# theori-io/nrsc5

Hardware: NVIDIA H100
Metric: cu8 I/Q Msamples/s (higher is better)
Workload: dtype u8/int16/f32

## Files before the change

### nrsc5_b200/csrc/common.cuh

```cuda
#pragma once
#include <cuda_runtime.h>
#include <stdint.h>

namespace nb {

constexpr int NFFT = 2048;
constexpr int NCP = 112;
constexpr int NSYM = NFFT + NCP;
constexpr int BLK = 32;
constexpr int NACQ = NSYM * (BLK + 1);
constexpr int LB0 = NFFT / 2 - 546;
constexpr int UB1 = NFFT / 2 + 546;
constexpr int PW = 19;
constexpr int MAXPART = 14;
constexpr int SIDE = MAXPART * PW + 1;
constexpr int NBINS = 2 * SIDE;
constexpr int PM_BLOCK = 23040;
constexpr int P1_LEN = 146176;
constexpr int P1_ENC = P1_LEN * 5 / 2;
constexpr int P1_VIT = P1_LEN * 3;
constexpr int P1_STEPS = P1_LEN + 64;
constexpr int PIDS_LEN = 80;
constexpr int P3_LEN = 4608;
constexpr int IV_N = 147456;
// ... 23 lines not shown
                   REC_BER = 6, REC_SOFT_PM = 8, REC_BLOCK = 9, REC_PAD = 12;

__host__ __device__ inline int compact_of_bin(int b)
{
    if (b >= LB0 && b < LB0 + SIDE) return b - LB0;
    if (b > UB1 - SIDE && b <= UB1) return SIDE + (b - (UB1 - SIDE + 1));
    return -1;
}

constexpr int L2_QUEUE = 40;

struct StreamState {
    long long in_avail;
    long long start;
    float prev_angle;
    float2 phase;
    int keep_extra;
    int cfo;
    int state;
    int samperr;
    float angle;
    int psmi, cfo_wait, bc, mer_cnt;
    float err_lb, err_ub;
    int started_pm;
    int active;
    int blk_samperr;
    int blk_state_in;
    int blk_go;
    float theta;
    float2 phase0;
    int p1_ready;
    int p1_slow;
    int p1_retry;
    unsigned p1_rec;
    unsigned p1_lost_rec;
    int p1_errs;
    int p1_done;
    int pids_pending;
    int pids_bc[16];
    unsigned pids_rec[16];
    long long px_total[2];
    int px_started[2];
    int xq_pending[PX_GROUPS];
    long long xq_k0[PX_GROUPS][P3_SLOTS];
    unsigned xq_rec[PX_GROUPS][P3_SLOTS];
    int force_state;
    int l2_n;
    unsigned l2_off[L2_QUEUE], l2_lc[L2_QUEUE], l2_nbits[L2_QUEUE];
    unsigned log_len;
    unsigned log_overflow;
    unsigned long long blocks_done;
    unsigned long long frames_done;
    unsigned long long p1_fallbacks;
    unsigned long long ph_cyc[6];
    unsigned long long ph_n[6];
    unsigned long long sy_cyc[6];
    short bp_hist[31][2];
    short bp_hist_next[31][2];
};

struct EngineDims {
    int nstreams;
    size_t in_stride;
    size_t log_cap;
    int emit_soft;
    int cs16;
    int px_enabled;
    int l2;
    int cluster;
};

struct PxBufs {
    int8_t *vin;
    uint2 *dec;
    uint32_t *spec, *end;
    int *endstate;
    uint2 *fspec, *fend;
    int *fhstate, *ftbend;
    uint32_t *bits;
    int *flags;
};

struct EngineCtl {
    unsigned long long progress;
    unsigned px_need;
    unsigned more;
};

struct StreamBrief {
    long long start;
    int state, bc, p1_ready, pad_;
};

struct DevPtrs {
    EngineCtl *ctl;
    StreamBrief *brief;
    const uint8_t *iq;
    StreamState *st;
    float *cfreq;
    float *cphase;
    float2 *nco;
    float2 *bins;
    int8_t *pm;
    short2 *ydec;
    float2 *acq_sums;
    float2 *tbuf;
    int8_t *vit_in;
    uint2 *vit_dec;
    uint32_t *p1_bits;
    uint2 *vspec, *vend;
    int *hstate, *tbend;
    uint32_t *v64_spec, *v64_end;
    int *v64_endstate;
    int8_t *px_ring[2];
    const uint32_t *iv_delay;
    const uint32_t *iv_delay_s;
    PxBufs xb[PX_GROUPS];
    uint8_t *log;
    const float *shape;
    const float2 *twid;
    const uint32_t *p1_lut;
    const uint8_t *pn;
    const uint32_t *pnw;
};

__device__ inline uint8_t *log_reserve(const DevPtrs &p, const EngineDims &d, int s, uint32_t type, uint32_t plen)
{
    StreamState &st = p.st[s];
    uint32_t need = 8 + ((plen + 3) & ~3u);
    if ((size_t)st.log_len + need > d.log_cap) {
        st.log_overflow = 1;
        return nullptr;
    }
    uint8_t *w = p.log + (size_t)s * d.log_cap + st.log_len;
    reinterpret_cast<uint32_t *>(w)[0] = type;
    reinterpret_cast<uint32_t *>(w)[1] = plen;
    st.log_len += need;
    return w + 8;
}

__device__ __forceinline__ void l2_enqueue(StreamState &st, int l2_on, unsigned off, unsigned lc, unsigned nbits)
{
    if (!l2_on) return;
    if (st.l2_n >= L2_QUEUE) {
        st.log_overflow = 1;
        return;
    }
    const int e = st.l2_n++;
    st.l2_off[e] = off;
    st.l2_lc[e] = lc;
    st.l2_nbits[e] = nbits;
}

template <int R>
__device__ __forceinline__ void halfband_run(const uint32_t *w, short2 *y)
{
    const int tap[4] = { -134, 1078, -4417, 19864 };
    int lr[R + 7], li[R + 7];
    int cr[R], ci[R];
#pragma unroll
    for (int q = 0; q < R + 7; q++) {
        const uint32_t v = w[q];
        lr[q] = (int)(v & 0xffu);
        li[q] = (int)((v >> 8) & 0xffu);
        if (q >= 3 && q < R + 3) {
            cr[q - 3] = (int)((v >> 16) & 0xffu);
            ci[q - 3] = (int)(v >> 24);
        }
    }
#pragma unroll
    for (int r = 0; r < R; r++) {
        int ar = cr[r] * 64 - 127 * 64, ai = ci[r] * 64 - 127 * 64;
#pragma unroll
        for (int k = 0; k < 4; k++) {
            ar += ((lr[r + k] + lr[r + 7 - k]) * tap[k] - 254 * tap[k]) >> 9;
            ai += ((li[r + k] + li[r + 7 - k]) * tap[k] - 254 * tap[k]) >> 9;
        }
        y[r] = make_short2((short)ar, (short)ai);
    }
}

}
```

### nrsc5_b200/csrc/front.cuh

```cuda
#pragma once
#include "pids_crc.cuh"
#include "common.cuh"
#include "fft.cuh"
#include "viterbi_pack.cuh"

namespace nb {

constexpr int FRONT_THREADS = 1024;
constexpr int TEAMS = FRONT_THREADS / 128;
constexpr int MAXREF = 15;
constexpr int IN_BYTES = 4 * NSYM + 28 + 16 + 16;
constexpr int IN_STRIDE = 8704;
constexpr int ACQ_TILE = 4096;

__device__ int g_dbg;

__constant__ int c_compat_mode[64];
__constant__ unsigned c_pn80[3];
__constant__ short c_bp_tap[32];

__device__ __forceinline__ float2 cmulf(float2 a, float2 b)
{
    return make_float2(a.x * b.x - a.y * b.y, a.x * b.y + a.y * b.x);
}
__device__ __forceinline__ float2 cexp_j(float a)
{
    float s, c;
    sincosf(a, &s, &c);
    return make_float2(c, s);
}

__device__ __forceinline__ int partitions_per_band(int psmi)
{
    switch (c_compat_mode[psmi & 63]) {
    case 2: return 11;
    case 3: return 12;
    case 5: case 6: case 11: return 14;
    default: return 10;
    }
}

__device__ void set_state(const DevPtrs &p, const EngineDims &d, int s, int ns)
{
    StreamState &st = p.st[s];
    if (st.state == ns) return;
    if (st.state == ST_FINE) log_reserve(p, d, s, REC_LOST_SYNC, 0);
    if (ns == ST_FINE) {
        float fo = (float)(((double)st.prev_angle - 2 * M_PI * st.cfo) * 744187.5 / (2 * M_PI * NFFT));
        uint8_t *w = log_reserve(p, d, s, REC_SYNC, 8);
        if (w) {
            reinterpret_cast<float *>(w)[0] = fo;
            reinterpret_cast<int *>(w)[1] = st.psmi;
        }
    }
    st.state = ns;
}

constexpr int DEMOD_RUN = 17;
constexpr int TEAM_SMEM = IN_STRIDE + NSYM * (int)sizeof(short2);
struct DemodSmem {
    float2 buf[TEAMS][TEAM_SMEM / sizeof(float2)];
    float2 symphase[TEAMS];
};
static_assert(FFT_SMEM_ELEMS * sizeof(float2) <= TEAM_SMEM && TEAM_SMEM % 16 == 0, "a team's FFT buffer");
static_assert(DEMOD_RUN * FFT_THREADS >= NSYM && DEMOD_RUN % 2 == 1, "a symbol's runs");
struct PrepSmem {
    uint32_t words[ACQ_TILE + 40];
    short2 ytile[ACQ_TILE + 32];
    float2 sums[NSYM];
    float red_mag[FRONT_THREADS];
    int red_idx[FRONT_THREADS];
    float2 red_v[FRONT_THREADS];
};
constexpr int ACQ1_RUN = 3;
constexpr int ACQ1_WORDS = (NSYM + 38 + 3 + 3) / 4 * 4;
static_assert(ACQ1_RUN * FRONT_THREADS >= NSYM + 31 && ACQ1_RUN % 2 == 1, "a tile's runs");
struct Acq1Smem {
    uint32_t words[2][ACQ1_WORDS];
    short2 ytile[NSYM + 32];
    float2 ring[2][NSYM];
    float2 sums[NSYM];
    float2 shape[NCP];
    float red_mag[FRONT_THREADS];
    int red_idx[FRONT_THREADS];
    float2 red_v[FRONT_THREADS];
};
struct PidsSmem {
    int8_t vit[PIDS_LEN * 3];
    uint2 dec[PIDS_LEN + 64];
};
constexpr int ZS = 32;
constexpr int EQ_LD = BLK + 1;
constexpr int EQ_MAXPART = 12;
constexpr int EQ_ROWS = 2 * EQ_MAXPART * (PW - 1);
struct SyncSmem {
    float phs[BLK][ZS];
    float2 eph[2 * MAXREF][BLK];
    float smag[2 * MAXREF];
    float cfq[2 * MAXREF];
    union {
        float2 eq[EQ_ROWS][EQ_LD];
        struct {
            int offs[76][22];
            int verdict[76];
            int winner;
        } srch;
    };
    float wred[FRONT_THREADS / 32][2];
    float fb_w[2][MAXREF], fb_xy[2][MAXREF + 1];
    float4 rowc[EQ_ROWS];
    int ref_ok[2 * MAXREF], ref_bc[2 * MAXREF], ref_psmi[2 * MAXREF];
    bool px_on[2];
    long long px_T[2];
    uint8_t *soft_w;
    int do_search;
};
struct FrontSmem {
    float2 tw[FFT_TW];
    float2 nco[NSYM];
    float2 zref[BLK][ZS];
    signed char ref_slot[NBINS + 2];
    uint8_t ref_mask[128];
    union {
        DemodSmem demod;
        PrepSmem prep;
        Acq1Smem acq1;
        SyncSmem sync;
        PidsSmem pidsq[16];
    } u;
};

__device__ void pids_decode_warp(const DevPtrs &p, const EngineDims &d, int s, int e, PidsSmem &sm, int lane)
{
    const StreamState &st = p.st[s];
    const int bc = st.pids_bc[e];
    const int8_t *pmall = p.pm + (size_t)s * 16 * PM_BLOCK;
    const int8_t PMV[20] = { 10, 2, 18, 6, 14, 8, 16, 0, 12, 4, 11, 3, 19, 7, 15, 9, 17, 1, 13, 5 };
    for (int o = lane; o < PIDS_LEN * 3; o += 32) {
        int8_t v = 0;
        if (o % 6 != 5) {
            unsigned i = (unsigned)bc * 200 + (unsigned)(o - o / 6);
            unsigned part = (unsigned)PMV[i % 20];
            unsigned block = i / 200;
            unsigned k = (i / 20) % 10 + P1_ENC / 320;
            unsigned row = (k * 11) % 32, col = (k * 11 + k / 288) % 36;
            v = pmall[(block * 32 + row) * 720 + part * 36 + col];
        }
        sm.vit[o] = v;
    }
    __syncwarp();
    const int l = lane & 15;
    VitHalf<false> vh;
    vh.init(l);
    vitc_run<false>(vh, sm.vit, PIDS_LEN, PIDS_LEN + 64, 0, PIDS_LEN + 64, 0, sm.dec, lane < 16, l);
    __syncwarp();
    int v = (short)(vh.E & 0xffff), state = 2 * l;
    const int w1 = (short)(vh.O & 0xffff);
    if (w1 > v) { v = w1; state = 2 * l + 1; }
    int v2 = (short)(vh.E >> 16), idx2 = 2 * l + 32;
    const int w3 = (short)(vh.O >> 16);
    if (w3 > v2) { v2 = w3; idx2 = 2 * l + 33; }
    if (v2 > v) { v = v2; state = idx2; }
#pragma unroll
    for (int o = 8; o; o >>= 1) {
        const int ov = __shfl_xor_sync(0xffffffffu, v, o, 16), oi = __shfl_xor_sync(0xffffffffu, state, o, 16);
        if (ov > v || (ov == v && oi < state)) { v = ov; state = oi; }
    }
    if (lane == 0) {
        uint8_t pk[10];
        for (int i = 0; i < 10; i++) pk[i] = 0;
        for (int q = PIDS_LEN + 63; q >= 0; q--) {
            if (q >= 32 && q < 32 + PIDS_LEN) {
                const int i = q - 32;
                const int bit = ((state >> 5) & 1) ^ (int)((c_pn80[i >> 5] >> (i & 31)) & 1u);
                pk[i >> 3] |= (uint8_t)(bit << (7 - (i & 7)));
            }
            state = vitc_prev_head(state, sm.dec, q);
        }
        if (st.pids_rec[e] != 0xffffffffu) {
            uint8_t *w = p.log + (size_t)s * d.log_cap + st.pids_rec[e];
            for (int i = 0; i < 10; i++) w[i] = pk[i];
            w[10] = (uint8_t)pids_crc12_ok(pk);
        }
    }
}

__device__ void front_pids_flush(const DevPtrs &p, const EngineDims &d, int s, PidsSmem *sm, int t)
{
    StreamState &st = p.st[s];
    const int n = st.pids_pending, warp = t >> 5;
    if (warp < n) pids_decode_warp(p, d, s, warp, sm[warp], t & 31);
    __syncthreads();
    if (t == 0) st.pids_pending = 0;
}

constexpr int ACQ_RUN = 5;
static_assert(ACQ_RUN * FRONT_THREADS >= ACQ_TILE + 31, "a tile's runs");
template <int RUN>
__device__ __forceinline__ void acq_tile_input(const EngineDims &d, const uint32_t *words, short2 *ytile, const StreamState &st,
                                               int i0, int L, int t)
{
    const int kb = i0 == 0 ? 31 : 0;
    if (t < kb) ytile[t] = make_short2(st.bp_hist[t][0], st.bp_hist[t][1]);
    const int n = L + 31 - kb;
    if (d.cs16) {
        for (int k = kb + t; k < L + 31; k += FRONT_THREADS) {
            const uint32_t w = words[k + 7];
            ytile[k] = make_short2((short)(w & 0xffff), (short)(w >> 16));
        }
    } else if (RUN * t < n) {
        const int k = kb + min(RUN * t, n - RUN);
        halfband_run<RUN>(words + k, ytile + k);
    }
}

__device__ __forceinline__ float2 acq_bandpass(const short2 *yy)
{
    short accr = 0, acci = 0;
#pragma unroll 5
    for (int k = 1; k < 16; k++) {
        const short2 a = yy[k], b = yy[32 - k];
        accr = (short)(accr + ((((int)a.x + (int)b.x) * c_bp_tap[k]) >> 15));
        acci = (short)(acci + ((((int)a.y + (int)b.y) * c_bp_tap[k]) >> 15));
    }
    const short2 c = yy[16];
    accr = (short)(accr + (((int)c.x * c_bp_tap[16]) >> 15));
    acci = (short)(acci + (((int)c.y * c_bp_tap[16]) >> 15));
    return make_float2(__fdiv_rn((float)accr, 32767.0f), __fdiv_rn((float)acci, -32767.0f));
}

__device__ __forceinline__ void fill_nco(const DevPtrs &p, float2 *nco, float theta, int t)
{
    for (int j = t; j < NSYM; j += FRONT_THREADS) {
        float2 e = cexp_j(theta * (float)j);
        if (j < NCP || j >= NFFT) {
            const float w = __ldg(&p.shape[j]);
            e = make_float2(e.x * w, e.y * w);
        }
        nco[j] = e;
    }
}

__device__ int front_prep_begin(const DevPtrs &p, const EngineDims &d, int s, int t)
{
    StreamState &st = p.st[s];
    __shared__ int sh_active;
    if (t == 0) {
        if (st.force_state >= 0) {
            set_state(p, d, s, st.force_state);
            st.force_state = -1;
        }
        const long long avail = *reinterpret_cast<volatile long long *>(&st.in_avail);
        int act = avail >= 2 * (st.start + NACQ);
        if (act && st.state == ST_FINE) {
            const int need = px_need_of(c_compat_mode[st.psmi & 63]);
            if (need & ~d.px_enabled) {
                atomicOr(&p.ctl->px_need, (unsigned)need);
                act = 0;
            }
        }
        st.active = act;
        sh_active = act ? (st.state == ST_FINE ? 1 : 2) : 0;
        if (act) atomicAdd(&p.ctl->progress, 1ull);
    }
    __syncthreads();
    const int mode = sh_active;
    __syncthreads();
    return mode;
}

__device__ void front_acq_tiles(const DevPtrs &p, const EngineDims &d, int s, PrepSmem &sm, int t, int rank, int nranks)
{
    StreamState &st = p.st[s];
    const uint8_t *iq = p.iq + (size_t)s * d.in_stride;
    float2 *tb = p.tbuf + (size_t)s * NACQ;
// ... 173 lines not shown
        const int woff = (int)((start - 38) & 3);
        static_assert(NSYM % 4 == 0, "tiles start at the same word phase");
        const int nvec = (woff + NSYM + 38 + 3) / 4;
        auto fetch = [&](int T) {
            const long long w0 = start + (long long)T * NSYM - 38;
            const long long w0a = w0 & ~3LL;
            uint4 *dst = reinterpret_cast<uint4 *>(sm.words[T & 1]);
            for (int v = t; v < nvec; v += FRONT_THREADS) {
                const long long a = w0a + 4 * v;
                if (a >= 0) {
#if defined(NB_EMU)
                    dst[v] = *reinterpret_cast<const uint4 *>(iq + 4 * a);
#else
                    asm volatile("cp.async.cg.shared.global [%0], [%1], 16;" ::"r"((unsigned)__cvta_generic_to_shared(dst + v)), "l"(iq + 4 * a) : "memory");
#endif
                } else {
                    const uint32_t z = d.cs16 ? 0u : 0x7f7f7f7fu;
                    dst[v] = make_uint4(z, z, z, z);
                }
            }
#if !defined(NB_EMU)
            asm volatile("cp.async.commit_group;" ::: "memory");
#endif
        };
        for (int i = t; i < NSYM; i += FRONT_THREADS) sm.sums[i] = make_float2(0.f, 0.f);
        if (t < NCP) sm.shape[t] = make_float2(__ldg(&p.shape[t]), __ldg(&p.shape[t + NFFT]));
        fetch(0);
#pragma unroll 1
        for (int T = 0; T <= NT; T++) {
            if (T + 1 < NT) fetch(T + 1);
#if !defined(NB_EMU)
            if (T + 1 < NT) asm volatile("cp.async.wait_group 1;" ::: "memory");
            else asm volatile("cp.async.wait_group 0;" ::: "memory");
#endif
            __syncthreads();
            if (T < NT) acq_tile_input<ACQ1_RUN>(d, sm.words[T & 1] + woff, sm.ytile, st, T * NSYM, NSYM, t);
            if (T >= 2) {
                const float2 *ya = sm.ring[T & 1], *yb = sm.ring[(T - 1) & 1];
                for (int i = t; i < NSYM; i += FRONT_THREADS) {
                    const float2 a = ya[i], b = i + NFFT < NSYM ? ya[i + NFFT] : yb[i + NFFT - NSYM];
                    const float2 pr = cmulf(a, make_float2(b.x, -b.y));
                    sm.sums[i].x += pr.x;
                    sm.sums[i].y += pr.y;
                }
            }
            __syncthreads();
            if (T < NT) {
                float2 *y = sm.ring[T & 1];
                for (int j = t; j < NSYM; j += FRONT_THREADS) y[j] = acq_bandpass(sm.ytile + j);
                if (T == NT - 1 && t < 31) {
                    const short2 v = sm.ytile[NSYM + t];
                    st.bp_hist[t][0] = v.x;
                    st.bp_hist[t][1] = v.y;
                }
            }
        }
        __syncthreads();
        float best = -1.0f;
        int besti = 0;
        float2 bestv = make_float2(0.f, 0.f);
        for (int i = t; i < NSYM; i += FRONT_THREADS) {
            float2 v = make_float2(0.f, 0.f);
            for (int j = 0; j < NCP; j++) {
                int q = i + j;
                if (q >= NSYM) q -= NSYM;
                const float2 sv = sm.sums[q];
                const float2 ab = sm.shape[j];
                v.x += (sv.x * ab.x) * ab.y;
                v.y += (sv.y * ab.x) * ab.y;
            }
            const float mag = v.x * v.x + v.y * v.y;
            if (mag > best) { best = mag; besti = i; bestv = v; }
        }
        sm.red_mag[t] = best; sm.red_idx[t] = besti; sm.red_v[t] = bestv;
        __syncthreads();
        for (int o = FRONT_THREADS / 2; o; o >>= 1) {
            if (t < o) {
                const float m2 = sm.red_mag[t + o];
                const int i2 = sm.red_idx[t + o];
                if (m2 > sm.red_mag[t] || (m2 == sm.red_mag[t] && i2 < sm.red_idx[t])) {
                    sm.red_mag[t] = m2; sm.red_idx[t] = i2; sm.red_v[t] = sm.red_v[t + o];
                }
            }
            __syncthreads();
        }
        if (t == 0) {
            const float2 w = cmulf(sm.red_v[0], cexp_j(-st.prev_angle));
            const float angle_diff = atan2f(w.y, w.x);
            const float factor = (st.prev_angle != 0.0f) ? 0.25f : 1.0f;
            const float angle = st.prev_angle + (angle_diff * factor);
            st.prev_angle = angle;
            sh_angle = angle;
            sh_samperr = (sm.red_idx[0] + NSYM - 15) % NSYM;
            if (st.state == ST_NONE) st.state = ST_COARSE;
        }
    } else if (t == 0) {
        sh_samperr = NSYM / 2 + st.samperr;
        st.samperr = 0;
        const float angle = st.prev_angle + (-st.angle);
        st.angle = 0;
        st.prev_angle = angle;
        sh_angle = angle;
    }
    __syncthreads();

    const int samperr = sh_samperr;
    const int adj = NSYM / 2 - samperr;
    if (adj != 0) {
        float *cp = p.cphase + (size_t)s * NFFT;
        for (int i = t; i < SIDE; i += FRONT_THREADS) {
            const int bl = LB0 + i, bu = UB1 - i;
            cp[bl] = (float)((double)cp[bl] - (double)(adj * (bl - NFFT / 2) * 2) * M_PI / NFFT);
            cp[bu] = (float)((double)cp[bu] - (double)(adj * (bu - NFFT / 2) * 2) * M_PI / NFFT);
        }
    }
    if (t == 0) {
        float angle = sh_angle;
        angle = (float)((double)angle - 2 * M_PI * st.cfo);
        const float pre = (float)(-adj) * angle / (float)NFFT;
        const float2 ph = cmulf(st.phase, cexp_j(pre));
        const float theta = angle / (float)NFFT;
        st.phase0 = ph;
        st.theta = theta;
        sh_theta = theta;
        st.blk_samperr = samperr;
        st.blk_state_in = state_in;
        double sn, cs;
        sincos((double)theta * (double)(NSYM * BLK), &sn, &cs);
        const float2 pe = cmulf(ph, make_float2((float)cs, (float)sn));
        const float nrm = sqrtf(pe.x * pe.x + pe.y * pe.y);
        st.phase = make_float2(pe.x / nrm, pe.y / nrm);
        uint8_t *w = log_reserve(p, d, s, REC_BLOCK, 32);
        if (w) {
            int *wi = reinterpret_cast<int *>(w);
            float *wf = reinterpret_cast<float *>(w);
            wi[0] = state_in; wi[1] = samperr; wf[2] = angle; wf[3] = ph.x; wf[4] = ph.y; wi[5] = st.cfo;
            wi[6] = (int)(unsigned)(st.start & 0xffffffffLL);
            wi[7] = (int)(st.start >> 32);
        }
    }
    __syncthreads();
    fill_nco(p, nco, sh_theta, t);
    __syncthreads();
    return true;
}

__device__ __forceinline__ float2 sample_q15(short2 h)
{
    const float sc = 1.0f / 32767.0f;
    return make_float2((float)h.x * sc, (float)h.y * -sc);
}

__device__ void front_demod(const DevPtrs &p, const EngineDims &d, int s, int sym, DemodSmem &sm, const float2 *nco,
                            const float2 *tw, float2 (*zref)[ZS], const signed char *ref_slot, const uint8_t *ref_mask,
                            int half, int tl, long long start, int samperr, float theta, float2 phase0)
{
    float2 *buf = sm.buf[half];
    uint8_t *in = reinterpret_cast<uint8_t *>(buf);
    const int bar = 1 + half;
    const long long base = start + samperr + (long long)NSYM * sym;
    const long long b0 = 4 * base - 28;
    const long long b0a = b0 & ~15LL;
    const int off = (int)(b0 - b0a);
    const uint8_t *iq = p.iq + (size_t)s * d.in_stride;
    bar_sync(bar);
    {
        const int nvec = (off + 4 * NSYM + 28 + 15) / 16;
        uint4 *dst = reinterpret_cast<uint4 *>(in);
        for (int v = tl; v < nvec; v += 128) {
            const long long a = b0a + 16LL * v;
            if (a >= 0) {
#if defined(NB_EMU)
                dst[v] = *reinterpret_cast<const uint4 *>(iq + a);
#else
                asm volatile("cp.async.cg.shared.global [%0], [%1], 16;" ::"r"((unsigned)__cvta_generic_to_shared(dst + v)), "l"(iq + a) : "memory");
#endif
            } else {
                dst[v] = make_uint4(0x7f7f7f7fu, 0x7f7f7f7fu, 0x7f7f7f7fu, 0x7f7f7f7fu);
            }
        }
#if !defined(NB_EMU)
        asm volatile("cp.async.commit_group;\n\tcp.async.wait_group 0;" ::: "memory");
#endif
    }
    if (tl == 0) {
        double sn, cs;
        sincos((double)theta * (double)(NSYM * sym), &sn, &cs);
        sm.symphase[half] = cmul(phase0, make_float2((float)cs, (float)sn));
    }
    bar_sync(bar);

    const uint32_t *sw = reinterpret_cast<const uint32_t *>(in + off);
    const short2 *y;
    if (d.cs16) {
        y = reinterpret_cast<const short2 *>(sw + 7);
    } else {
        short2 *yw = reinterpret_cast<short2 *>(in + IN_STRIDE);
        const int j0 = min(DEMOD_RUN * tl, NSYM - DEMOD_RUN);
        halfband_run<DEMOD_RUN>(sw + j0, yw + j0);
        y = yw;
        bar_sync(bar);
    }
    float2 v[16];
    v[0] = cmul(sample_q15(y[tl]), nco[tl]);
    if (tl < NCP) {
        const int j = NFFT + tl;
        v[0] = cadd(v[0], cmul(sample_q15(y[j]), nco[j]));
    }
#pragma unroll
    for (int n1 = 1; n1 < 16; n1++) {
        const int j = n1 * 128 + tl;
        v[n1] = cmul(sample_q15(y[j]), nco[j]);
    }
    bar_sync(bar);
    float2 out[2][8];
    fft2048_block<true>(v, out, buf, tw, tl, bar);
    const float2 sp = sm.symphase[half];

    float2 *dst = p.bins + ((size_t)s * BLK + sym) * NBINS;
    float2 *zr = zref[sym];
    const unsigned mask = ref_mask[tl];
    auto put = [&](int c, float2 v, int bit) {
        dst[c] = v;
        if (mask & (1u << bit)) zr[ref_slot[c]] = v;
    };
#pragma unroll
    for (int h = 0; h < 2; h++) {
        const int q = tl + 128 * h;
        if (q >= 222) put(q - 222, cmul(out[h][5], sp), 4 * h);
        if (q <= 232) put(q + 34, cmul(out[h][6], sp), 4 * h + 1);
        if (q >= 24) put(q + 243, cmul(out[h][1], sp), 4 * h + 2);
        if (q <= 34) put(q + 499, cmul(out[h][2], sp), 4 * h + 3);
    }
}

__device__ __forceinline__ int ref_bin(int slot)
{
    return slot < MAXREF ? LB0 + PW * slot : UB1 - PW * (slot - MAXREF);
}

__device__ __forceinline__ float atan2_short(float y, float x)
{
    const float ax = fabsf(x), ay = fabsf(y);
    const float mx = fmaxf(ax, ay), mn = fminf(ax, ay);
    const float t = mx > 0.f ? __fdividef(mn, mx) : 0.f;
    const float z = t * t;
    float p = 0.0028340641874819994f;
    p = __fmaf_rn(p, z, -0.016005029901862144f);
    p = __fmaf_rn(p, z, 0.042587608098983765f);
    p = __fmaf_rn(p, z, -0.07495445758104324f);
    p = __fmaf_rn(p, z, 0.10636754333972931f);
    p = __fmaf_rn(p, z, -0.14202570915222168f);
    p = __fmaf_rn(p, z, 0.19992484152317047f);
    p = __fmaf_rn(p, z, -0.3333306610584259f);
    p = __fmaf_rn(p, z, 1.0f);
    float r = p * t;
    if (ay > ax) r = 1.57079637f - r;
    if (x < 0.f) r = 3.14159274f - r;
    return copysignf(r, y);
}

__device__ __forceinline__ void costas_row(float2 *z, float *phs, int zs, float &cfreq, float &cphase, int cfo, float alpha, float beta, bool FAST)
{
    const unsigned pat_pos = (1u << 1) | (1u << 5) | (1u << 6) | (1u << 8) | (1u << 21);
    const unsigned pat_neg = (1u << 0) | (1u << 2) | (1u << 3) | (1u << 4) | (1u << 9) | (1u << 13) | (1u << 14) | (1u << 20) |
                             (1u << 22) | (1u << 31);
    const float cfo_freq = (float)(2 * M_PI * cfo * NCP / NFFT);
    const float PI_F = 3.14159274101257324f;
    const float TWO_PI_HI = 6.28318548202514648f, TWO_PI_LO = -1.74845553e-07f;
    float f = cfreq, ph = cphase;
#pragma unroll 1
    for (int n = 0; n < BLK; n++) {
        const float2 v = z[n * zs];
        float2 rot;
        if (FAST) {
            float sn, cs;
            __sincosf(-ph, &sn, &cs);
            rot = make_float2(cs, sn);
        } else {
            rot = cexp_j(-ph);
        }
        const float2 u = cmulf(v, rot);
        const float error = (FAST ? atan2_short((u.x * u.y) * 2.0f, u.x * u.x - u.y * u.y)
                                  : atan2f((u.x * u.y) * 2.0f, u.x * u.x - u.y * u.y)) * 0.5f;
        phs[n * zs] = ph;
        z[n * zs] = u;
        f += beta * error;
        if (f > 0.5f) f = 0.5f;
        if (f < -0.5f) f = -0.5f;
        ph += (f + cfo_freq) + (alpha * error);
        if (ph >= PI_F) ph = (ph - TWO_PI_HI) - TWO_PI_LO;
        if (ph <= -PI_F) ph = (ph + TWO_PI_HI) + TWO_PI_LO;
    }
    float x = 0;
#pragma unroll 4
    for (int n = 0; n < BLK; n++) x += z[n * zs].x * (float)((int)((pat_pos >> n) & 1u) - (int)((pat_neg >> n) & 1u));
    if (x < 0) {
#pragma unroll 4
        for (int n = 0; n < BLK; n++) {
            phs[n * zs] = (float)((double)phs[n * zs] + M_PI);
            z[n * zs] = make_float2(z[n * zs].x * -1.0f, z[n * zs].y * -1.0f);
        }
        ph = (float)((double)ph + M_PI);
    }
    cfreq = f;
    cphase = ph;
}

__device__ __forceinline__ int needle_bit(int n, unsigned rsid)
{
    const signed char base[BLK] = { 0, 1, 0, 0, 0, 1, 1, -1, 1, 0, 0, 0, -1, 0, 0, -1,
                                    -1, -1, -1, -1, 0, 1, 0, -1, -1, -1, -1, -1, -1, -1, -1, 0 };
    if (n == 10) return (int)(rsid >> 1);
    if (n == 11) return (int)((rsid >> 1) ^ (rsid & 1));
    return base[n];
}

__device__ int ref_find(const float2 *z, int zs, unsigned rsid)
{
    unsigned raw = 0;
    for (int n = 0; n < BLK; n++)
        if (!(z[n * zs].x <= 0)) raw |= 1u << n;
    for (int pass = 0; pass < 2; pass++) {
        for (int n = 0; n < BLK; n++) {
            int i;
            for (i = 0; i < BLK; i++) {
                const int nb_ = needle_bit(i, rsid);
                if (nb_ < 0) continue;
                if (nb_ != (int)((raw >> ((n + i) & 31)) & 1)) break;
            }
            if (i == BLK) return n;
        }
        raw = ~raw;
    }
    return -1;
}

__device__ __forceinline__ float half_pi_wrap(float a, float b)
{
    float dd = a - b;
    while ((double)dd > M_PI / 2) dd = (float)((double)dd - M_PI);
    while ((double)dd < -M_PI / 2) dd = (float)((double)dd + M_PI);
    return dd;
}

__device__ __forceinline__ int8_t soft_demap(float x, float mult)
{
    const float v = fmaxf(fminf(x, 1.0f), -1.0f) * mult;
    int r = __float2int_rz(v);
    const float f = v - (float)r;
    if (f >= 0.5f) r++;
    else if (f <= -0.5f) r--;
    return (int8_t)r;
}

template <bool CL>
__device__ void front_sync(const DevPtrs &p, const EngineDims &d, int s, SyncSmem &sm, float2 (*zref)[ZS], int t)
{
    StreamState &st = p.st[s];
    float *cfreq = p.cfreq + (size_t)s * NFFT;
    float *cphase = p.cphase + (size_t)s * NFFT;
    float2 *bins = p.bins + (size_t)s * BLK * NBINS;
    auto ldbin = [](const float2 *q) -> float2 { return CL ? __ldcg(q) : *q; };
    const float loop_bw = 0.05f, damping = 0.70710678f;
    const float denom = 1 + (2 * damping * loop_bw) + (loop_bw * loop_bw);
    const float alpha = (4 * damping * loop_bw) / denom, beta = (4 * loop_bw * loop_bw) / denom;

    int ppb = partitions_per_band(st.psmi);
    int nref = ppb + 1;
    long long sy0 = clock64();
    const bool sy_on = st.state == ST_FINE;
    auto sylap = [&](int k) {
        if (t == 0 && sy_on) {
            const long long c1 = clock64();
            st.sy_cyc[k] += (unsigned long long)(c1 - sy0);
            sy0 = c1;
        }
// ... 305 lines not shown
                    } else {
                        const int ci = (sb == 0 ? PW * i : (NBINS - 1 - PW) - PW * i) + 1 + 2 * c4;
                        a = ldbin(&bins[(size_t)n * NBINS + ci]);
                        b = ldbin(&bins[(size_t)n * NBINS + ci + 1]);
                    }
                    const float ml = mult[lower_scale_only ? 0 : sb];
                    const unsigned w = (unsigned)(uint8_t)soft_demap(a.x, ml) | ((unsigned)(uint8_t)soft_demap(a.y, ml) << 8) |
                                       ((unsigned)(uint8_t)soft_demap(b.x, ml) << 16) | ((unsigned)(uint8_t)soft_demap(b.y, ml) << 24);
                    const long long pos = (T + n * per_sym + q * 36 + 4 * c4) % PX_RING;
                    *reinterpret_cast<uint32_t *>(ring + pos) = w;
                }
            };
            if (sm.px_on[0]) px_demap(p.px_ring[0] + (size_t)s * PX_RING, sm.px_T[0], cm == 2 ? 2 : 4, 10, false);
            if (sm.px_on[1]) px_demap(p.px_ring[1] + (size_t)s * PX_RING, sm.px_T[1], 4, 12, true);
        } else if (t >= 32) {
            const int lane = t & 31;
            if (lane < ppb) {
                sm.fb_w[0][lane] = half_pi_wrap(sm.phs[0][lane], sm.phs[0][lane + 1]);
                sm.fb_w[1][lane] = half_pi_wrap(sm.phs[0][MAXREF + lane + 1], sm.phs[0][MAXREF + lane]);
            }
            if (lane <= ppb) {
                sm.fb_xy[0][lane] = (float)(LB0 + PW * lane - NFFT / 2) * sm.cfq[lane];
                sm.fb_xy[1][lane] = (float)(UB1 - PW * lane - NFFT / 2) * sm.cfq[MAXREF + lane];
            }
            __syncwarp();
            float fb_angle = 0;
            if (lane == 31) {
                float samperr = 0, angle = 0, sum_xy = 0, sum_x2 = 0;
                for (int i = 0; i < ppb; i++) {
                    samperr += sm.fb_w[0][i];
                    samperr += sm.fb_w[1][i];
                }
                const double inv_2pi = 1.0 / (2 * M_PI);
                samperr = (float)((double)(samperr / (float)(ppb * 2) * (float)NFFT / (float)PW) * inv_2pi);
                for (int i = 0; i <= ppb; i++) {
                    float x;
                    x = (float)(LB0 + PW * i - NFFT / 2);
                    angle += sm.cfq[i]; sum_xy += sm.fb_xy[0][i]; sum_x2 += x * x;
                    x = (float)(UB1 - PW * i - NFFT / 2);
                    angle += sm.cfq[MAXREF + i]; sum_xy += sm.fb_xy[1][i]; sum_x2 += x * x;
                }
                samperr = (float)((double)samperr - (double)((sum_xy / sum_x2) * (float)NFFT) * inv_2pi * BLK);
                st.samperr = (int)roundf(samperr);
                angle /= (float)((ppb + 1) * 2);
                st.angle = angle;
                fb_angle = angle;
            }
            fb_angle = __shfl_sync(0xffffffffu, fb_angle, 31);
            const int i = lane < MAXREF ? lane : lane - MAXREF;
            if (lane < 2 * MAXREF && i < nref) cfreq[ref_bin(lane)] = sm.cfq[lane] - fb_angle;
        } else if (t == 0) {
            st.err_lb += e_sb[0];
            st.err_ub += e_sb[1];
            if (++st.mer_cnt == 16) {
                const float signal = (float)(2 * BLK * (ppb * 18) * st.mer_cnt);
                uint8_t *w = log_reserve(p, d, s, REC_MER, 8);
                if (w) {
                    reinterpret_cast<float *>(w)[0] = 10 * log10f(signal / st.err_lb);
                    reinterpret_cast<float *>(w)[1] = 10 * log10f(signal / st.err_ub);
                }
                st.mer_cnt = 0;
                st.err_lb = 0;
                st.err_ub = 0;
            }
            if (d.emit_soft) {
                sm.soft_w = log_reserve(p, d, s, REC_SOFT_PM, 4 + PM_BLOCK);
                if (sm.soft_w) *reinterpret_cast<uint32_t *>(sm.soft_w) = (uint32_t)bc;
            }
            uint8_t *w = log_reserve(p, d, s, REC_PIDS, 11);
            const int e = st.pids_pending;
            st.pids_rec[e] = w ? (unsigned)(w - (p.log + (size_t)s * d.log_cap)) : 0xffffffffu;
            st.pids_bc[e] = bc;
            st.pids_pending = e + 1;
            if (bc == 0) st.started_pm = 1;
            unsigned lost_slot = 0xffffffffu;
            if (st.started_pm && bc == 15) {
                const unsigned len0 = st.log_len;
                uint8_t *bw = log_reserve(p, d, s, REC_BER, 4);
                uint8_t *fw = bw ? log_reserve(p, d, s, REC_FRAME, 8 + P1_LEN / 8) : nullptr;
                if (!fw) { st.log_len = len0; bw = nullptr; }
                st.p1_rec = (bw && fw) ? (unsigned)(bw - (p.log + (size_t)s * d.log_cap)) : 0xffffffffu;
                if (fw) {
                    reinterpret_cast<uint32_t *>(fw)[0] = 0;
                    reinterpret_cast<uint32_t *>(fw)[1] = P1_LEN;
                    uint8_t *lw = log_reserve(p, d, s, REC_PAD, 0);
                    if (lw) lost_slot = (unsigned)(lw - 8 - (p.log + (size_t)s * d.log_cap));
                }
                st.p1_lost_rec = lost_slot;
                l2_enqueue(st, d.l2, st.p1_rec != 0xffffffffu ? st.p1_rec + 4 + 8 + 8 : 0xffffffffu, 0, P1_LEN);
                st.p1_ready = 1;
            }
#pragma unroll
            for (int g = 0; g < PX_GROUPS; g++) {
                const PxGroup x = px_group(g);
                if (!(x.modes >> cm & 1)) continue;
                if ((bc & 1) == 0) st.px_started[x.ring] = 1;
                if (!st.px_started[x.ring]) continue;
                st.px_total[x.ring] += x.len;
                const long long k0 = st.px_total[x.ring] - 2 * x.len;
                if ((bc & 1) && k0 >= 32 * x.len && st.xq_pending[g] < P3_SLOTS) {
                    uint8_t *fw = log_reserve(p, d, s, REC_FRAME, 8 + x.len / 8);
                    const int e = st.xq_pending[g];
                    st.xq_k0[g][e] = k0;
                    st.xq_rec[g][e] = fw ? (unsigned)(fw - (p.log + (size_t)s * d.log_cap)) : 0xffffffffu;
                    if (fw) {
                        reinterpret_cast<uint32_t *>(fw)[0] = x.lc;
                        reinterpret_cast<uint32_t *>(fw)[1] = x.len;
                    }
                    l2_enqueue(st, d.l2, fw ? st.xq_rec[g][e] + 8 : 0xffffffffu, x.lc, x.len);
                    st.xq_pending[g] = e + 1;
                }
            }
            if (lost_slot != 0xffffffffu && st.log_len == lost_slot + 8) {
                st.log_len = lost_slot;
                st.p1_lost_rec = 0xffffffffu;
            }
            st.bc = (bc + 1) % 16;
        }
        __syncthreads();
        if (d.emit_soft && sm.soft_w)
            for (int o = t; o < PM_BLOCK; o += FRONT_THREADS) sm.soft_w[4 + o] = (uint8_t)pm[o];
    }
    if (t == 0) {
        const int keep = NSYM + (NSYM / 2 - st.blk_samperr) + st.keep_extra;
        st.keep_extra = 0;
        st.start += NACQ - keep;
        st.blocks_done++;
    }
    sylap(5);
}

__device__ __forceinline__ void cluster_barrier()
{
#if defined(NB_EMU)
#else
    asm volatile("barrier.cluster.arrive.release.aligned;\n\tbarrier.cluster.wait.acquire.aligned;" ::: "memory");
#endif
}

template <bool CL>
__global__ void __launch_bounds__(FRONT_THREADS, 1) k_stream(DevPtrs p, EngineDims d, int max_blocks, int last_pass)
{
#if defined(NB_EMU)
    unsigned char *front_smem_raw = emu::dyn_smem();
#else
    extern __shared__ __align__(16) unsigned char front_smem_raw[];
#endif
    FrontSmem &sm = *reinterpret_cast<FrontSmem *>(front_smem_raw);
    const int t = threadIdx.x, team = t >> 7, tl = t & 127;
    const int C = CL ? d.cluster : 1;
    const int s = (int)blockIdx.x / C, rank = (int)blockIdx.x % C;
    StreamState &st = p.st[s];
    for (int i = t; i < FFT_TW; i += FRONT_THREADS) sm.tw[i] = __ldg(&p.twid[i]);
    for (int c = t; c < NBINS; c += FRONT_THREADS)
        sm.ref_slot[c] = c < SIDE ? (c % PW == 0 ? c / PW : -1) : ((NBINS - 1 - c) % PW == 0 ? MAXREF + (NBINS - 1 - c) / PW : -1);
    if (t < 128) {
        unsigned m = 0;
        for (int h = 0; h < 2; h++) {
            const int q = t + 128 * h;
            const int c[4] = { q >= 222 ? q - 222 : -1, q <= 232 ? q + 34 : -1, q >= 24 ? q + 243 : -1, q <= 34 ? q + 499 : -1 };
            for (int k = 0; k < 4; k++)
                if (c[k] >= 0 && (c[k] < SIDE ? c[k] % PW == 0 : (NBINS - 1 - c[k]) % PW == 0)) m |= 1u << (4 * h + k);
        }
        sm.ref_mask[t] = (uint8_t)m;
    }
    __syncthreads();

    const bool owner = !CL || rank == 0;
    if (max_blocks > 16) max_blocks = 16;
    if (owner && t == 0) {
        for (int g = 0; g < PX_GROUPS; g++) st.xq_pending[g] = 0;
    }
    __syncthreads();
    for (int nb = 0;; nb++) {
        long long c0 = clock64();
        auto lap = [&](int ph) {
            if (owner && t == 0) {
                const long long c1 = clock64();
                st.ph_cyc[ph] += (unsigned long long)(c1 - c0);
                st.ph_n[ph]++;
                c0 = c1;
            }
        };
        int mode = 0;
        if (!CL) {
            if (nb < max_blocks && !st.p1_ready) mode = front_prep_single(p, d, s, sm.u.acq1, sm.nco, t) ? 1 : 0;
            if (mode == 0) break;
        } else {
            if (owner) {
                if (nb < max_blocks && !st.p1_ready) mode = front_prep_begin(p, d, s, t);
                if (mode == 1) front_prep_finish(p, d, s, sm.u.prep, sm.nco, t, 1);
            }
            if (owner && t == 0) {
                st.blk_go = mode;
                __threadfence();
            }
            cluster_barrier();
            if (!owner) mode = __ldcg(&st.blk_go);
            if (mode == 0) break;
            if (mode == 2) {
                front_acq_tiles(p, d, s, sm.u.prep, t, rank, C);
                __threadfence();
                cluster_barrier();
                front_acq_corr(p, s, t, rank, C);
                __threadfence();
                cluster_barrier();
                if (owner) {
                    front_prep_finish(p, d, s, sm.u.prep, sm.nco, t, 2);
                    __threadfence();
                }
                cluster_barrier();
            }
        }
        lap(st.blk_state_in == ST_FINE ? 2 : 1);
        const long long start = CL ? __ldcg(&st.start) : st.start;
        const int samperr = CL ? __ldcg(&st.blk_samperr) : st.blk_samperr;
        const float theta = CL ? __ldcg(&st.theta) : st.theta;
        const float2 phase0 = CL ? __ldcg(&st.phase0) : st.phase0;
        if (CL && !owner) {
            fill_nco(p, sm.nco, theta, t);
            __syncthreads();
        }
#pragma unroll 1
        for (int pass = 0; pass < BLK / (TEAMS * C); pass++)
            front_demod(p, d, s, (pass * C + rank) * TEAMS + team, sm.u.demod, sm.nco, sm.tw, sm.zref, sm.ref_slot, sm.ref_mask, team, tl, start, samperr, theta, phase0);
        if (CL) {
            __threadfence();
            cluster_barrier();
        }
        if (CL && !owner) continue;
        __syncthreads();
        lap(3);
        front_sync<CL>(p, d, s, sm.u.sync, sm.zref, t);
        __syncthreads();
        lap(st.blk_state_in == ST_FINE ? 4 : 5);
    }
    if (CL && !owner) return;
    __syncthreads();
    if (st.pids_pending) {
        const long long c0 = clock64();
        front_pids_flush(p, d, s, sm.u.pidsq, t);
        if (t == 0) {
            st.ph_cyc[0] += (unsigned long long)(clock64() - c0);
            st.ph_n[0]++;
        }
    }
    if (t == 0) {
        StreamBrief b;
        b.start = st.start;
        b.state = st.state;
        b.bc = st.bc;
        b.p1_ready = st.p1_ready;
        b.pad_ = 0;
        p.brief[s] = b;
        const long long avail = *reinterpret_cast<volatile long long *>(&st.in_avail);
        if (last_pass && avail >= 2 * (st.start + NACQ)) atomicAdd(&p.ctl->more, 1u);
    }
}

}
```

Before: 158,200.

## Use dp2a for halfband filter, unroll symbol copy loop, pack reference plan

The halfband decimator now loads raw packed u8 words and computes the tap sums with dp2a instructions and byte_perm pairing, replacing per-byte extraction and scalar multiplies. The per-symbol cp.async copy loop is fully unrolled into five fixed iterations with precomputed source and destination pointers. The reference-pilot scatter drops the per-bin slot table and bitmask in favour of one byte per thread that encodes the single slot and position. Together these aim to cut integer ALU and shared-memory lookups in the front-end demod, at the cost of relying on each thread touching at most one reference bin.

```diff
diff --git a/nrsc5_b200/csrc/common.cuh b/nrsc5_b200/csrc/common.cuh
--- a/nrsc5_b200/csrc/common.cuh
+++ b/nrsc5_b200/csrc/common.cuh
@@ -199,29 +199,36 @@
     st.l2_nbits[e] = nbits;
 }
 
+template <bool HI>
+__device__ __forceinline__ int dp2a_su(int a, uint32_t b, int c)
+{
+#if defined(NB_EMU)
+    const int s = HI ? 16 : 0;
+    return c + (int)(short)(a & 0xffff) * (int)((b >> s) & 0xffu) + (int)(short)(a >> 16) * (int)((b >> (s + 8)) & 0xffu);
+#else
+    int d;
+    if (HI) asm("dp2a.hi.s32.u32 %0, %1, %2, %3;" : "=r"(d) : "r"(a), "r"(b), "r"(c));
+    else    asm("dp2a.lo.s32.u32 %0, %1, %2, %3;" : "=r"(d) : "r"(a), "r"(b), "r"(c));
+    return d;
+#endif
+}
+
 template <int R>
 __device__ __forceinline__ void halfband_run(const uint32_t *w, short2 *y)
 {
     const int tap[4] = { -134, 1078, -4417, 19864 };
-    int lr[R + 7], li[R + 7];
-    int cr[R], ci[R];
+    uint32_t v[R + 7];
 #pragma unroll
-    for (int q = 0; q < R + 7; q++) {
-        const uint32_t v = w[q];
-        lr[q] = (int)(v & 0xffu);
-        li[q] = (int)((v >> 8) & 0xffu);
-        if (q >= 3 && q < R + 3) {
-            cr[q - 3] = (int)((v >> 16) & 0xffu);
-            ci[q - 3] = (int)(v >> 24);
-        }
-    }
+    for (int q = 0; q < R + 7; q++) v[q] = w[q];
 #pragma unroll
     for (int r = 0; r < R; r++) {
-        int ar = cr[r] * 64 - 127 * 64, ai = ci[r] * 64 - 127 * 64;
+        int ar = dp2a_su<true>(64, v[r + 3], -127 * 64), ai = dp2a_su<true>(64 << 16, v[r + 3], -127 * 64);
 #pragma unroll
         for (int k = 0; k < 4; k++) {
-            ar += ((lr[r + k] + lr[r + 7 - k]) * tap[k] - 254 * tap[k]) >> 9;
-            ai += ((li[r + k] + li[r + 7 - k]) * tap[k] - 254 * tap[k]) >> 9;
+            const uint32_t pr = __byte_perm(v[r + k], v[r + 7 - k], 0x5140);
+            const int tt = (tap[k] & 0xffff) | (tap[k] << 16);
+            ar += dp2a_su<false>(tt, pr, -254 * tap[k]) >> 9;
+            ai += dp2a_su<true>(tt, pr, -254 * tap[k]) >> 9;
         }
         y[r] = make_short2((short)ar, (short)ai);
     }
diff --git a/nrsc5_b200/csrc/front.cuh b/nrsc5_b200/csrc/front.cuh
--- a/nrsc5_b200/csrc/front.cuh
+++ b/nrsc5_b200/csrc/front.cuh
@@ -90,6 +90,7 @@
     uint2 dec[PIDS_LEN + 64];
 };
 constexpr int ZS = 32;
+static_assert(2 * MAXREF <= 32, "a reference slot fits the 5 bits of FrontSmem::ref_plan");
 constexpr int EQ_LD = BLK + 1;
 constexpr int EQ_MAXPART = 12;
 constexpr int EQ_ROWS = 2 * EQ_MAXPART * (PW - 1);
@@ -119,8 +120,7 @@
     float2 tw[FFT_TW];
     float2 nco[NSYM];
     float2 zref[BLK][ZS];
-    signed char ref_slot[NBINS + 2];
-    uint8_t ref_mask[128];
+    uint8_t ref_plan[128];
     union {
         DemodSmem demod;
         PrepSmem prep;
@@ -600,7 +600,7 @@
 }
 
 __device__ void front_demod(const DevPtrs &p, const EngineDims &d, int s, int sym, DemodSmem &sm, const float2 *nco,
-                            const float2 *tw, float2 (*zref)[ZS], const signed char *ref_slot, const uint8_t *ref_mask,
+                            const float2 *tw, float2 (*zref)[ZS], const uint8_t *ref_plan,
                             int half, int tl, long long start, int samperr, float theta, float2 phase0)
 {
     float2 *buf = sm.buf[half];
@@ -614,17 +614,21 @@
     bar_sync(bar);
     {
         const int nvec = (off + 4 * NSYM + 28 + 15) / 16;
-        uint4 *dst = reinterpret_cast<uint4 *>(in);
-        for (int v = tl; v < nvec; v += 128) {
-            const long long a = b0a + 16LL * v;
-            if (a >= 0) {
+        static_assert(4 * 128 < (4 * NSYM + 28 + 15) / 16 && (12 + 4 * NSYM + 28 + 15) / 16 <= 5 * 128, "a symbol's copies");
+        uint4 *dst = reinterpret_cast<uint4 *>(in) + tl;
+        const uint8_t *src = iq + b0a + 16 * tl;
+        const bool head = b0a < 0;
+#pragma unroll
+        for (int i = 0; i < 5; i++) {
+            if (i == 4 && tl + 4 * 128 >= nvec) break;
+            if (!head || b0a + 16 * (tl + 128 * i) >= 0) {
 #if defined(NB_EMU)
-                dst[v] = *reinterpret_cast<const uint4 *>(iq + a);
+                dst[128 * i] = *reinterpret_cast<const uint4 *>(src + 2048 * i);
 #else
-                asm volatile("cp.async.cg.shared.global [%0], [%1], 16;" ::"r"((unsigned)__cvta_generic_to_shared(dst + v)), "l"(iq + a) : "memory");
+                asm volatile("cp.async.cg.shared.global [%0], [%1], 16;" ::"r"((unsigned)__cvta_generic_to_shared(dst + 128 * i)), "l"(src + 2048 * i) : "memory");
 #endif
             } else {
-                dst[v] = make_uint4(0x7f7f7f7fu, 0x7f7f7f7fu, 0x7f7f7f7fu, 0x7f7f7f7fu);
+                dst[128 * i] = make_uint4(0x7f7f7f7fu, 0x7f7f7f7fu, 0x7f7f7f7fu, 0x7f7f7f7fu);
             }
         }
 #if !defined(NB_EMU)
@@ -666,11 +670,12 @@
     const float2 sp = sm.symphase[half];
 
     float2 *dst = p.bins + ((size_t)s * BLK + sym) * NBINS;
-    float2 *zr = zref[sym];
-    const unsigned mask = ref_mask[tl];
-    auto put = [&](int c, float2 v, int bit) {
+    const unsigned plan = ref_plan[tl];
+    float2 *zp = zref[sym] + (plan & 31u);
+    const unsigned pk = plan >> 5;
+    auto put = [&](int c, float2 v, unsigned k) {
         dst[c] = v;
-        if (mask & (1u << bit)) zr[ref_slot[c]] = v;
+        if (pk == k) *zp = v;
     };
 #pragma unroll
     for (int h = 0; h < 2; h++) {
@@ -1282,17 +1287,19 @@
     const int s = (int)blockIdx.x / C, rank = (int)blockIdx.x % C;
     StreamState &st = p.st[s];
     for (int i = t; i < FFT_TW; i += FRONT_THREADS) sm.tw[i] = __ldg(&p.twid[i]);
-    for (int c = t; c < NBINS; c += FRONT_THREADS)
-        sm.ref_slot[c] = c < SIDE ? (c % PW == 0 ? c / PW : -1) : ((NBINS - 1 - c) % PW == 0 ? MAXREF + (NBINS - 1 - c) / PW : -1);
     if (t < 128) {
-        unsigned m = 0;
+        unsigned m = 0xffu;
         for (int h = 0; h < 2; h++) {
             const int q = t + 128 * h;
             const int c[4] = { q >= 222 ? q - 222 : -1, q <= 232 ? q + 34 : -1, q >= 24 ? q + 243 : -1, q <= 34 ? q + 499 : -1 };
-            for (int k = 0; k < 4; k++)
-                if (c[k] >= 0 && (c[k] < SIDE ? c[k] % PW == 0 : (NBINS - 1 - c[k]) % PW == 0)) m |= 1u << (4 * h + k);
-        }
-        sm.ref_mask[t] = (uint8_t)m;
+            for (int k = 0; k < 4; k++) {
+                if (c[k] < 0) continue;
+                const int slot = c[k] < SIDE ? (c[k] % PW == 0 ? c[k] / PW : -1)
+                                             : ((NBINS - 1 - c[k]) % PW == 0 ? MAXREF + (NBINS - 1 - c[k]) / PW : -1);
+                if (slot >= 0) m = (unsigned)(4 * h + k) << 5 | (unsigned)slot;
+            }
+        }
+        sm.ref_plan[t] = (uint8_t)m;
     }
     __syncthreads();
 
@@ -1353,7 +1360,7 @@
         }
 #pragma unroll 1
         for (int pass = 0; pass < BLK / (TEAMS * C); pass++)
-            front_demod(p, d, s, (pass * C + rank) * TEAMS + team, sm.u.demod, sm.nco, sm.tw, sm.zref, sm.ref_slot, sm.ref_mask, team, tl, start, samperr, theta, phase0);
+            front_demod(p, d, s, (pass * C + rank) * TEAMS + team, sm.u.demod, sm.nco, sm.tw, sm.zref, sm.ref_plan, team, tl, start, samperr, theta, phase0);
         if (CL) {
             __threadfence();
             cluster_barrier();
```

New measurement: 166,300, median of 6. 5.1% higher.
